# youliangtan/tennisbot-rl

Measured on AMD Instinct MI355X. Metric: env steps/sec (whole node), SwingRacket-v0 @4096 envs/GPU, higher is better.
Workload: dtype f32

## Files before the change

include/tb_stepper.h:

```cpp
#ifndef TB_STEPPER_H
#define TB_STEPPER_H

#include <stddef.h>
#include <stdint.h>

#ifdef __cplusplus
extern "C" {
#endif

#define TB_ABI_VERSION 4

#define TB_OK 0
#define TB_E_INVAL (-1)
#define TB_E_NODEVICE (-2)
#define TB_E_PARAMS (-3)
#define TB_E_UNSUPPORTED (-4)
#define TB_E_TIMEOUT (-5)

#define TB_ENV_SWING 0
#define TB_ENV_TENNIS 1

#define TB_SWING_ACT_DIM 6
#define TB_SWING_OBS_DIM 6
#define TB_TENNIS_ACT_DIM 2
// ... 220 lines not shown
                   long long n_rows, const int64_t *idx_dev, int batch, const float *actor_dev, const float *target_dev,
                   const float *log_ent_coef_dev, const float *eps_next_dev, float gamma, float *y_dev, void *workspace_dev,
                   size_t workspace_bytes);
int tb_tqc_critic_grad(int env_kind, int device, void *stream, const float *obs_dev, const float *action_dev, long long n_rows,
                       const int64_t *idx_dev, int batch, const float *critic_dev, const float *y_dev, float *grad_dev,
                       double *stats_dev, void *workspace_dev, size_t workspace_bytes);
int tb_tqc_actor_grad(int env_kind, int device, void *stream, int batch, const float *actor_dev, const float *critic_dev,
                      const float *log_ent_coef_dev, const float *eps_dev, float *actor_grad_dev, float *ent_grad_dev,
                      double *stats_dev, void *workspace_dev, size_t workspace_bytes);

int tb_set_pipeline(TbHandle *h, int enable);
int tb_flush(TbHandle *h, void *stream);
#define TB_MAX_MARKS 64
int tb_mark_enable(TbHandle *h, int on);
int tb_mark_record(TbHandle *h, int k, void *stream);
int tb_mark_begin(TbHandle *h);
int tb_mark_host_wait(TbHandle *h, int k, int timeout_ms);
long long tb_mark_count(TbHandle *h, int k);
int tb_pipeline_sync(TbHandle *h, int host_wait);
int tb_phase(TbHandle *h);
int tb_phase_advance(TbHandle *h, int n_steps);
int tb_pipeline_form(TbHandle *h);
int tb_step_waves(TbHandle *h);
int tb_pipeline_recover(TbHandle *h);

int tb_get_state(TbHandle *h, uint32_t *words, uint8_t *done, int on_device, void *stream);
int tb_set_state(TbHandle *h, const uint32_t *words, const uint8_t *done, int on_device, void *stream);

#define TB_N_COUNTERS 9
int tb_counters(TbHandle *h, uint64_t *out, void *stream);
int tb_counters_reset(TbHandle *h, void *stream);
int tb_sealed_substeps(TbHandle *h, uint64_t *out, void *stream);

int tb_diag_stream_copy(const uint32_t *src_dev, uint32_t *dst_dev, int n, int rows, int device, void *stream);
int tb_diag_idle(int waves, int microseconds, int device, void *stream);
int tb_diag_two_wave_gate(TbHandle *h, uint8_t *out_dev, void *stream);
int tb_diag_fail_alloc(int nth);

#ifdef __cplusplus
}
#endif
#endif
```

tennisbot_rl_amd/csrc/tb_es.hpp:

```cpp
#pragma once

namespace {

template <int KIND> struct EsNet {
  static constexpr int O = Dims<KIND>::O, A = Dims<KIND>::A, C0 = 8, C1 = 12;
  static constexpr int W0 = 0, B0 = W0 + C0 * O * 2, G0W = B0 + C0, G0B = G0W + C0 * O * 2;
  static constexpr int W1 = G0B + C0, B1 = W1 + C1 * C0 * 2, G1W = B1 + C1, G1B = G1W + C1 * C0 * 2;
  static constexpr int W2 = G1B + C1, B2 = W2 + A * C1 * 2, P = B2 + A;
  static constexpr int PP = (P + 3) / 4 * 4;
  static constexpr int R_X = 0, R_H0 = O, R_H1 = O + 3 * C0, RING = O + 3 * C0 + 5 * C1;
};
template <int KIND> constexpr int es_floats() { return EsNet<KIND>::P; }
static_assert(EsNet<TB_ENV_SWING>::P == 766 && EsNet<TB_ENV_TENNIS>::P == 858, "GatedCNN parameter counts of the reference");
constexpr int TB_ES_LDS_MEMBERS = 8;

constexpr bool es_rows_in_registers(int kind, bool rg) { return kind == TB_ENV_TENNIS && !rg; }
constexpr int es_lds_words(int kind, bool rg) { return lds_words(!es_rows_in_registers(kind, rg), rg); }

struct EsArgs {
  const float* weights;
  size_t stride;
  int per_member;
  double* ret;
  int32_t* len;
// ... 95 lines not shown
  }
  stage_hull(s_hull, A.hull, A.P.n_hull);
  __syncthreads();
  const int m = (live ? i : last) / E.per_member;
  const float* W = staged ? s_w + (m - m0) * N::PP : E.weights + (size_t)m * E.stride;
  float* ring = s_ring + lane;

  EnvRegs e;
  idle_env(e);
  if (live) load_env<KIND>(A.words, A.done_state, A.n, i, e);
  Manifold M;
  init_manifold(M, lane, 64, !es_rows_in_registers(KIND, RG));
  uint32_t cnt[TB_N_COUNTERS] = {};
  KParams Pl = A.P;
  double nrm = 0.0, mean[NO], mdiff[NO];
#pragma unroll
  for (int k = 0; k < NO; ++k) { mean[k] = 0.0; mdiff[k] = 0.0; }
  float o[NO];
  make_obs<KIND>(e, o);
  bool active = live;
  double ret = 0.0;
  int len = 0;
  constexpr unsigned FORM = (RG ? SF_RG : 0u) | SF_COLD | SF_WIDE | (es_rows_in_registers(KIND, RG) ? SF_REGROWS : 0u);
  for (int t = 0; t < T_MAX && __ballot(active) != 0ull; ++t) {
    float a[NA];
#pragma unroll
    for (int k = 0; k < NA; ++k) a[k] = 0.0f;
    const bool rec = active && t < E.t_max;
    if (active) {
      float x[NO], raw[NA];
      es_normalise<NO>(nrm, mean, mdiff, o, x);
      es_net_step<KIND>(W, x, ring, t, raw);
#pragma unroll
      for (int k = 0; k < NA; ++k) a[k] = clip_action(raw[k]);
      if (rec) {
        const size_t row = (size_t)t * A.n + i;
#pragma unroll
        for (int k = 0; k < NO; ++k) { E.t_net_in[row * NO + k] = x[k]; E.t_obs[row * NO + k] = o[k]; }
#pragma unroll
        for (int k = 0; k < NA; ++k) { E.t_act[row * NA + k] = a[k]; E.t_raw[row * NA + k] = raw[k]; }
      }
    }
    int ns = 1;
    bool d = false, parked = false;
    float rew;
    if (KIND == TB_ENV_SWING) rew = swing_step<FORM>(Pl, s_hull, e, M, a, ns, cnt, true, parked TB_STAMP_PASS);
    else rew = tennis_step<FORM>(Pl, s_hull, e, M, a, o, d, cnt TB_STAMP_PASS);
    if (active) {
      end_agent_step<KIND, RG, false>(A, i, e, M, parked, ns, (size_t)i, o, d, cnt);
      if (parked) rew = 0.0f;
      else ret += (double)rew;
      len = t + 1;
      if (rec) {
        E.t_rew[(size_t)t * A.n + i] = rew;
        E.t_done[(size_t)t * A.n + i] = d ? 1 : 0;
      }
      if (d) {
        cnt[5]++;
        active = false;
        idle_env(e);
        M.n = 0; M.deep = 0;
      }
    }
  }
  if (live) { E.ret[i] = ret; E.len[i] = len; }
  flush_counters(A.counters, cnt);
}

__global__ void __launch_bounds__(256) tb_es_fold_kernel(const float* rew_last, double* ret, int n, float* t_rew) {
  const int i = blockIdx.x * blockDim.x + threadIdx.x;
  if (i >= n) return;
  const float r = rew_last[i];
  ret[i] += (double)r;
  if (t_rew) t_rew[(size_t)25 * n + i] = r;
}

}
```

tennisbot_rl_amd/csrc/tb_kernels.hpp:

```cpp
#pragma once
#include <hip/hip_runtime.h>
#include <math.h>

#include "../../include/tb_stepper.h"
#include "tb_device.hpp"
using namespace tb;

namespace {

#define TB_COUNTER_SHARDS 64

struct KArgs {
  KParams P;
  uint32_t* words;
  uint8_t* done_state;
  const float4* hull;
  const float* actions;
  float* obs;
  float* reward;
  uint8_t* done_out;
  float* term_obs;
  int32_t* substeps;
  const uint8_t* mask;
  unsigned long long* counters;
// ... 41 lines not shown
}

template <int KIND> struct Dims;
template <> struct Dims<TB_ENV_SWING> { static constexpr int W = TB_SWING_WORDS, A = TB_SWING_ACT_DIM, O = TB_SWING_OBS_DIM, NAUX = 6; };
template <> struct Dims<TB_ENV_TENNIS> { static constexpr int W = TB_TENNIS_WORDS, A = TB_TENNIS_ACT_DIM, O = TB_TENNIS_OBS_DIM, NAUX = 4; };

template <bool OFF32>
TB_DEV uint32_t row_word(const uint32_t* w, int row, int n, int i) {
  if constexpr (OFF32) {
    const uint32_t byte = ((uint32_t)row * (uint32_t)n + (uint32_t)i) * 4u;
    return *reinterpret_cast<const uint32_t*>(reinterpret_cast<const char*>(w) + byte);
  } else return w[(size_t)row * n + i];
}
template <bool OFF32>
TB_DEV void row_store(uint32_t* w, int row, int n, int i, uint32_t v) {
  if constexpr (OFF32) {
    const uint32_t byte = ((uint32_t)row * (uint32_t)n + (uint32_t)i) * 4u;
    *reinterpret_cast<uint32_t*>(reinterpret_cast<char*>(w) + byte) = v;
  } else w[(size_t)row * n + i] = v;
}
template <int KIND> constexpr bool off32() { return KIND == TB_ENV_SWING; }
template <int KIND> TB_DEV float ld(const uint32_t* w, int row, int n, int i) { return __uint_as_float(row_word<off32<KIND>()>(w, row, n, i)); }
template <int KIND> TB_DEV void st(uint32_t* w, int row, int n, int i, float v) { row_store<off32<KIND>()>(w, row, n, i, __float_as_uint(v)); }

template <int KIND>
TB_DEV void load_env(const uint32_t* w, const uint8_t* done_state, int n, int i, EnvRegs& e) {
  e.r.p = mk(ld<KIND>(w, TB_W_RP, n, i), ld<KIND>(w, TB_W_RP + 1, n, i), ld<KIND>(w, TB_W_RP + 2, n, i));
  e.r.q.x = ld<KIND>(w, TB_W_RQ, n, i); e.r.q.y = ld<KIND>(w, TB_W_RQ + 1, n, i); e.r.q.z = ld<KIND>(w, TB_W_RQ + 2, n, i); e.r.q.w = ld<KIND>(w, TB_W_RQ + 3, n, i);
  e.r.v = mk(ld<KIND>(w, TB_W_RV, n, i), ld<KIND>(w, TB_W_RV + 1, n, i), ld<KIND>(w, TB_W_RV + 2, n, i));
  e.r.w = mk(ld<KIND>(w, TB_W_RW, n, i), ld<KIND>(w, TB_W_RW + 1, n, i), ld<KIND>(w, TB_W_RW + 2, n, i));
  e.b.p = mk(ld<KIND>(w, TB_W_BP, n, i), ld<KIND>(w, TB_W_BP + 1, n, i), ld<KIND>(w, TB_W_BP + 2, n, i));
  e.b.v = mk(ld<KIND>(w, TB_W_BV, n, i), ld<KIND>(w, TB_W_BV + 1, n, i), ld<KIND>(w, TB_W_BV + 2, n, i));
  e.b.w = mk(ld<KIND>(w, TB_W_BW, n, i), ld<KIND>(w, TB_W_BW + 1, n, i), ld<KIND>(w, TB_W_BW + 2, n, i));
#pragma unroll
  for (int k = 0; k < 6; ++k) e.aux[k] = k < Dims<KIND>::NAUX ? ld<KIND>(w, 22 + k, n, i) : 0.0f;
  e.step_count = (int)row_word<off32<KIND>()>(w, Dims<KIND>::W - 2, n, i);
  e.episode = row_word<off32<KIND>()>(w, Dims<KIND>::W - 1, n, i);
  e.done = done_state[i];
}

template <int KIND>
TB_DEV void store_env(uint32_t* w, uint8_t* done_state, int n, int i, const EnvRegs& e, bool all) {
  st<KIND>(w, TB_W_RP, n, i, e.r.p.x); st<KIND>(w, TB_W_RP + 1, n, i, e.r.p.y); st<KIND>(w, TB_W_RP + 2, n, i, e.r.p.z);
  st<KIND>(w, TB_W_RQ, n, i, e.r.q.x); st<KIND>(w, TB_W_RQ + 1, n, i, e.r.q.y); st<KIND>(w, TB_W_RQ + 2, n, i, e.r.q.z); st<KIND>(w, TB_W_RQ + 3, n, i, e.r.q.w);
  st<KIND>(w, TB_W_RV, n, i, e.r.v.x); st<KIND>(w, TB_W_RV + 1, n, i, e.r.v.y); st<KIND>(w, TB_W_RV + 2, n, i, e.r.v.z);
  st<KIND>(w, TB_W_RW, n, i, e.r.w.x); st<KIND>(w, TB_W_RW + 1, n, i, e.r.w.y); st<KIND>(w, TB_W_RW + 2, n, i, e.r.w.z);
// ... 394 lines not shown

TB_DEV void load_ball_side(const uint32_t* w, const uint8_t* done_state, int n, int i, EnvRegs& e) {
  constexpr int K = TB_ENV_SWING;
  e.r.p = mk(ld<K>(w, TB_W_RP, n, i), ld<K>(w, TB_W_RP + 1, n, i), ld<K>(w, TB_W_RP + 2, n, i));
  e.r.q.x = ld<K>(w, TB_W_RQ, n, i); e.r.q.y = ld<K>(w, TB_W_RQ + 1, n, i); e.r.q.z = ld<K>(w, TB_W_RQ + 2, n, i); e.r.q.w = ld<K>(w, TB_W_RQ + 3, n, i);
  e.b.p = mk(ld<K>(w, TB_W_BP, n, i), ld<K>(w, TB_W_BP + 1, n, i), ld<K>(w, TB_W_BP + 2, n, i));
  e.b.v = mk(ld<K>(w, TB_W_BV, n, i), ld<K>(w, TB_W_BV + 1, n, i), ld<K>(w, TB_W_BV + 2, n, i));
  e.b.w = mk(ld<K>(w, TB_W_BW, n, i), ld<K>(w, TB_W_BW + 1, n, i), ld<K>(w, TB_W_BW + 2, n, i));
  e.aux[0] = ld<K>(w, 22, n, i); e.aux[1] = ld<K>(w, 23, n, i);
  e.step_count = (int)row_word<true>(w, Dims<K>::W - 2, n, i);
  e.done = done_state[i];
}
TB_DEV bool two_wave_rare(const KParams& P, const EnvRegs& e) {
  bool rare = e.done != TB_DONE_NO || e.step_count >= 25;
  const vec3 d = e.b.p - e.r.p;
  if ((P.flags & TB_F_RACKET_BALL) && racket_in_reach(P, d, 1.0f)) {
    vec3 ql;
    float qax;
    rare |= racket_slab<false>(P, rotate_inv(e.r.q, d), 1.0f, ql, qax);
  }
  rare |= !(ball_low_point(P, e.b) >= P.static_top + 1.0e-3f);
  return rare;
}
TB_DEV bool two_wave_step(const KArgs& A, const EnvRegs& e, const float* a, int i, bool live TB_DIAG_T0_ARG) {
  constexpr int K = TB_ENV_SWING;
  const KParams& P = A.P;
  const bool racket_wave = threadIdx.x < 64;
  const int lane = (int)(threadIdx.x & 63);
  __shared__ float2 s_rp[64];
  __shared__ float s_ball_fin[64];
  __shared__ int s_rare;
  [[maybe_unused]] const int mk0 = racket_wave ? 0 : 8;
  TB_DIAG_WAIT_LOADS(live);
  TB_DIAG_MARK(mk0);
  if (__any(live && (e.done != TB_DONE_NO || e.step_count >= 25))) return false;
  if (racket_wave) {
    TB_DIAG_MARK(mk0 + 1);
    Racket r = e.r;
    const vec3 F = mk(a[0] * 400.0f, a[1] * 400.0f, FMA(a[2], 400.0f, 4.0f * 9.81f));
    const vec3 T = mk(a[3] * 5.0f, a[4] * 5.0f, a[5] * 5.0f);
    const float speed_r = sqrtf(dot(r.v, r.v));
    racket_velocity(P, r, F, T, rotate_inv(r.q, r.w), speed_r);
    r.p = fma3(P.dt, r.v, r.p);
    s_rp[lane] = make_float2(r.p.x, r.p.y);
    racket_orientation(P, r);
    TB_DIAG_MARK(mk0 + 2);
    asm volatile("s_waitcnt lgkmcnt(0)\n\ts_barrier" ::: "memory");
    TB_DIAG_MARK(mk0 + 3);
    if (__builtin_amdgcn_readfirstlane(s_rare)) return false;
    uint32_t cnt[TB_N_COUNTERS] = {};
    if (live) {
      st<K>(A.words, TB_W_RP, A.n, i, r.p.x); st<K>(A.words, TB_W_RP + 1, A.n, i, r.p.y); st<K>(A.words, TB_W_RP + 2, A.n, i, r.p.z);
      st<K>(A.words, TB_W_RQ, A.n, i, r.q.x); st<K>(A.words, TB_W_RQ + 1, A.n, i, r.q.y); st<K>(A.words, TB_W_RQ + 2, A.n, i, r.q.z);
      st<K>(A.words, TB_W_RQ + 3, A.n, i, r.q.w);
      st<K>(A.words, TB_W_RV, A.n, i, r.v.x); st<K>(A.words, TB_W_RV + 1, A.n, i, r.v.y); st<K>(A.words, TB_W_RV + 2, A.n, i, r.v.z);
      st<K>(A.words, TB_W_RW, A.n, i, r.w.x); st<K>(A.words, TB_W_RW + 1, A.n, i, r.w.y); st<K>(A.words, TB_W_RW + 2, A.n, i, r.w.z);
      float a0 = r.p.x * 0.0f, a1 = r.p.y * 0.0f, a2 = r.p.z * 0.0f, a3 = r.q.x * 0.0f;
      a0 = FMA(r.q.y, 0.0f, a0); a1 = FMA(r.q.z, 0.0f, a1); a2 = FMA(r.q.w, 0.0f, a2); a3 = FMA(r.v.x, 0.0f, a3);
      a0 = FMA(r.v.y, 0.0f, a0); a1 = FMA(r.v.z, 0.0f, a1); a2 = FMA(r.w.x, 0.0f, a2); a3 = FMA(r.w.y, 0.0f, a3);
      a0 = FMA(r.w.z, 0.0f, a0);
      const float t = (a0 + a1) + (a2 + a3);
      if (!(t == t && s_ball_fin[lane] != 0.0f)) cnt[7]++;
    }
    flush_counters(A.counters, cnt);
    TB_DIAG_MARK(mk0 + 4);
  } else {
    Ball b = e.b;
    const float speed_b = sqrtf(dot(b.v, b.v)), spin_b = sqrtf(dot(b.w, b.w));
    ball_velocity(P, b, mk(0.0f, 0.0f, 0.0f), speed_b, spin_b);
    b.p = fma3(P.dt, b.v, b.p);
    float a0 = b.p.x * 0.0f, a1 = b.p.y * 0.0f, a2 = b.p.z * 0.0f, a3 = b.v.x * 0.0f;
    a0 = FMA(b.v.y, 0.0f, a0); a1 = FMA(b.v.z, 0.0f, a1); a2 = FMA(b.w.x, 0.0f, a2); a3 = FMA(b.w.y, 0.0f, a3);
    a0 = FMA(b.w.z, 0.0f, a0);
    const float t = (a0 + a1) + (a2 + a3);
    s_ball_fin[lane] = t == t ? 1.0f : 0.0f;
    const bool rare = __any(live && two_wave_rare(P, e));
    if (lane == 0) s_rare = rare ? 1 : 0;
    TB_DIAG_MARK(mk0 + 1);
    TB_DIAG_MARK(mk0 + 2);
    asm volatile("s_waitcnt lgkmcnt(0)\n\ts_barrier" ::: "memory");
    TB_DIAG_MARK(mk0 + 3);
    if (rare) return false;
    if (live) {
      st<K>(A.words, TB_W_BP, A.n, i, b.p.x); st<K>(A.words, TB_W_BP + 1, A.n, i, b.p.y); st<K>(A.words, TB_W_BP + 2, A.n, i, b.p.z);
      st<K>(A.words, TB_W_BV, A.n, i, b.v.x); st<K>(A.words, TB_W_BV + 1, A.n, i, b.v.y); st<K>(A.words, TB_W_BV + 2, A.n, i, b.v.z);
      st<K>(A.words, TB_W_BW, A.n, i, b.w.x); st<K>(A.words, TB_W_BW + 1, A.n, i, b.w.y); st<K>(A.words, TB_W_BW + 2, A.n, i, b.w.z);
      row_store<true>(A.words, Dims<K>::W - 2, A.n, i, (uint32_t)(e.step_count + 1));
      float2* o = reinterpret_cast<float2*>(A.obs + (size_t)i * 6);
      o[0] = s_rp[lane]; o[1] = make_float2(b.p.x, b.p.y); o[2] = make_float2(e.aux[0], e.aux[1]);
      A.reward[i] = 0.0f;
      A.done_out[i] = 0;
      if (A.substeps) A.substeps[i] = 1;
    }
    TB_DIAG_MARK(mk0 + 4);
  }
  TB_DIAG_ADD_LANE0(mk0 + 5, 1);
  return true;
}

__global__ void __launch_bounds__(64) tb_diag_two_wave_gate_kernel(KArgs A, uint8_t* out) {
  const int i = blockIdx.x * 64 + threadIdx.x;
  if (i >= A.n) return;
  EnvRegs e;
  load_env<TB_ENV_SWING>(A.words, A.done_state, A.n, i, e);
  out[i] = two_wave_rare(A.P, e) ? 1 : 0;
}

}
#include "tb_policy.hpp"
namespace {

#ifndef TB_HINT_TENNIS_CONSTANTS
#define TB_HINT_TENNIS_CONSTANTS 1
#endif
#ifndef TB_HINT_TENNIS_OUTPUTS
#define TB_HINT_TENNIS_OUTPUTS 1
#endif
#ifndef TB_HINT_POLICY_VGPR_PARAMS
#define TB_HINT_POLICY_VGPR_PARAMS 1
#endif
constexpr bool step_rows_in_registers(int kind, bool lean, bool multi, bool rg, bool policy) { return !rg && (kind == TB_ENV_TENNIS || (lean && !multi && !policy)); }
constexpr bool step_has_two_waves(int kind, bool lean, bool multi, bool rg, bool policy) { return kind == TB_ENV_SWING && lean && !multi && !rg && !policy; }
constexpr int step_lds_words(int kind, bool lean, bool multi, bool rg, bool policy) { return lds_words(!step_rows_in_registers(kind, lean, multi, rg, policy), rg); }
template <int KIND, bool LEAN, bool MULTI, bool RG, bool POLICY = false, bool TWO_WAVE = false, int NET = TB_NET_DEFAULT>
__global__ void __launch_bounds__(256) tb_step_kernel(const uint32_t* __restrict__ k_words, const uint8_t* __restrict__ k_done, const float* __restrict__ k_actions,
                                                      const float4* __restrict__ k_hull, int k_n, int k_nhull, KArgs A) {
  constexpr int NA = Dims<KIND>::A, NO = Dims<KIND>::O;
  constexpr bool TABLE_IN_MEMORY = !POLICY && !MULTI && KIND == TB_ENV_TENNIS;
  static_assert(!TWO_WAVE || step_has_two_waves(KIND, LEAN, MULTI, RG, POLICY), "the two-wave form is the pipelined SwingRacket one-step kernel's");
  constexpr bool REGROWS = step_rows_in_registers(KIND, LEAN, MULTI, RG, POLICY);
  constexpr bool LAZYTAB = !POLICY && !MULTI && KIND == TB_ENV_SWING && LEAN && !RG;
  constexpr unsigned FORM = (RG ? SF_RG : 0u) | (REGROWS ? SF_REGROWS : 0u) | (LAZYTAB ? SF_LAZYTAB : 0u);
  __shared__ float4 s_lds_hull[TABLE_IN_MEMORY ? 1 : TB_HULL_LDS];
  __shared__ __attribute__((aligned(16))) float s_mean[POLICY ? 64 * 8 : 4];
  const int i = POLICY || TWO_WAVE ? blockIdx.x * 64 + (threadIdx.x & 63) : blockIdx.x * blockDim.x + threadIdx.x;
  constexpr bool SEP = KIND == TB_ENV_TENNIS;
  const uint32_t* __restrict__ w_words = SEP ? k_words : A.words;
  const uint8_t* __restrict__ w_done = SEP ? k_done : A.done_state;
  const float* __restrict__ w_actions = SEP ? k_actions : A.actions;
  const float4* __restrict__ w_hull = SEP ? k_hull : A.hull;
  const int w_n = SEP ? k_n : A.n, w_nhull = SEP ? k_nhull : A.P.n_hull;
  const float4* const s_hull = TABLE_IN_MEMORY ? w_hull : s_lds_hull;
  const bool live = i < w_n;
  EnvRegs e;
  TB_DIAG_NOW(t_entry);
  TB_DIAG_TRACE_ENTRY(trace_slot);
  TB_DIAG_CADENCE_ENTRY(cad_t0, cad_n);
  float a[NA];
  if (live && !(POLICY && threadIdx.x >= 64)) {
    if (TWO_WAVE && threadIdx.x >= 64) {
      load_ball_side(w_words, w_done, w_n, i, e);
    } else {
      load_env<KIND>(w_words, w_done, w_n, i, e);
      if (!POLICY) load_actions<KIND>(w_actions, (size_t)i, a);
    }
  }
  if constexpr (TWO_WAVE) {
    if (two_wave_step(A, e, a, i, live TB_DIAG_T0_PASS)) {
      TB_DIAG_TRACE_EXIT(trace_slot);
      TB_DIAG_CADENCE_EXIT(cad_t0, cad_n);
      return;
    }
    if (threadIdx.x >= 64) return;
  }
#if TB_HINT_TENNIS_CONSTANTS
  if constexpr (KIND == TB_ENV_TENNIS && !POLICY && !MULTI) {
    asm volatile("" :: "s"(A.P.dt), "s"(A.P.gravity), "s"(A.P.lin_damp), "s"(A.P.lin_damp_quad), "s"(A.P.racket_inv_mass), "s"(A.P.ball_inv_mass),
                 "s"(A.P.hull_bound_radius), "s"(A.P.hull_margin), "s"(A.P.ball_radius), "s"(A.P.contact_threshold), "s"(A.P.static_top), "s"(A.P.max_ang_step));
  }
#endif
#if TB_HINT_TENNIS_OUTPUTS
  if constexpr (KIND == TB_ENV_TENNIS && !POLICY && !MULTI)
    asm volatile("" :: "s"(A.obs), "s"(A.reward), "s"(A.done_out), "s"(A.substeps));
#endif
  Manifold M;
  init_manifold(M, POLICY ? (int)(threadIdx.x & 63) : (int)threadIdx.x, POLICY ? 64 : (int)blockDim.x, !REGROWS);
  const bool had_contacts = load_contacts<RG>(A, i, live && !(POLICY && threadIdx.x >= 64), M);
  if (POLICY) {
    static_assert(TB_HULL_LDS <= 256, "one outline row per thread");
    const bool has_row = (int)threadIdx.x < 2 * w_nhull || ((int)threadIdx.x >= TB_HULL_PLANES && (int)threadIdx.x < TB_HULL_LDS);
    float4 row = make_float4(0.0f, 0.0f, 0.0f, 0.0f);
    if (has_row) row = w_hull[threadIdx.x];
    policy_towers<KIND, NET>(A, s_mean);
    if (has_row) s_lds_hull[threadIdx.x] = row;
    __syncthreads();
    if (threadIdx.x >= 64) return;
// ... 37 lines not shown
      }
      write_obs<KIND>(A.obs, row, o);
      A.reward[row] = rew;
      A.done_out[row] = d ? 1 : 0;
      if constexpr (MULTI && !POLICY) {
        if (t + 1 < n_steps) {
#pragma unroll
          for (int k = 0; k < NA; ++k) a[k] = a_next[k];
        }
      }
    }
    TB_DIAG_ADD_LANE0(15, stamp_now() - t_loaded);
    if (A.substeps) A.substeps[i] = ns_total;
    save_env<KIND, RG>(A, i, e, M, any_reset, had_contacts);
  }
  TB_DIAG_ADD_LANE0(7, t_loaded - t_entry);
  flush_counters(A.counters, cnt);
  TB_DIAG_STAMPS_END(st);
  TB_DIAG_ADD_LANE0(8, stamp_now() - t_kernel0);
  TB_DIAG_ADD_LANE0(9, 1);
  TB_DIAG_ADD_LANE0(14, __builtin_amdgcn_s_memrealtime() - rt_kernel0);
  TB_DIAG_TRACE_EXIT(trace_slot);
  TB_DIAG_CADENCE_EXIT(cad_t0, cad_n);
}

constexpr bool policy_rollout_rows_in_registers(int kind) { return kind == TB_ENV_TENNIS; }
TB_DEV void idle_env(EnvRegs& e) {
  const vec3 z3 = mk(0.0f, 0.0f, 0.0f);
  e.r.p = mk(0.0f, 0.0f, 10.0f); e.r.q.x = 0.0f; e.r.q.y = 0.0f; e.r.q.z = 0.0f; e.r.q.w = 1.0f; e.r.v = z3; e.r.w = z3;
  e.b.p = mk(100.0f, 100.0f, 1000.0f); e.b.v = z3; e.b.w = z3;
#pragma unroll
  for (int k = 0; k < 6; ++k) e.aux[k] = 0.0f;
  e.aux[3] = 1.0f;
  e.aux[5] = 1.0f;
  e.step_count = -(1 << 30); e.episode = 0u; e.done = TB_DONE_NO;
}
constexpr int policy_rollout_lds_words(int kind, bool rg) { return lds_words(!policy_rollout_rows_in_registers(kind), rg); }
template <int KIND, int S, bool RG, int NET = TB_NET_DEFAULT>
__global__ void __launch_bounds__((2 * S + 1) * 64) tb_policy_rollout_kernel(KArgs A) {
  constexpr int NA = Dims<KIND>::A, NO = Dims<KIND>::O, E = TB_POLICY_SLICE * S;
  __shared__ float4 s_hull[TB_HULL_LDS];
  __shared__ __attribute__((aligned(16))) float s_mean[E * 8];
  __shared__ __attribute__((aligned(16))) float s_obs[E * NO];
  const int wave = threadIdx.x >> 6, lane = threadIdx.x & 63;
  stage_hull(s_hull, A.hull, A.P.n_hull);
  if (wave < 2 * S) {
// ... 129 lines not shown
    make_obs<KIND>(e, o);
    if (live) {
#pragma unroll
      for (int k = 0; k < NO; ++k) s_obs[lane * NO + k] = o[k];
    }
  }
  __syncthreads();
  float stdv[NA], lstd[NA];
#pragma unroll
  for (int k = 0; k < NA; ++k) { lstd[k] = A.pol_weights[PolicyBlob<KIND, NET>::LOG_STD + k]; stdv[k] = expf(lstd[k]); }
  KParams Pl = A.P;
#if TB_HINT_POLICY_VGPR_PARAMS
#define TB_PIN(f) asm volatile("" : "+v"(Pl.f))
  TB_PIN(dt); TB_PIN(gravity); TB_PIN(lin_damp); TB_PIN(ang_damp); TB_PIN(lin_damp_quad); TB_PIN(ang_damp_quad); TB_PIN(max_ang_step); TB_PIN(contact_threshold);
  TB_PIN(racket_inv_mass); TB_PIN(racket_inertia[0]); TB_PIN(racket_inertia[1]); TB_PIN(racket_inertia[2]);
  TB_PIN(racket_inv_inertia[0]); TB_PIN(racket_inv_inertia[1]); TB_PIN(racket_inv_inertia[2]);
  TB_PIN(racket_half_thick); TB_PIN(hull_margin); TB_PIN(hull_bound_radius); TB_PIN(ball_inv_mass); TB_PIN(ball_radius); TB_PIN(magnus_k); TB_PIN(static_top);
#undef TB_PIN
#endif
  bool active = live;
  double ret = 0.0;
  int len = 0;
  constexpr unsigned FORM = (RG ? SF_RG : 0u) | SF_COLD | SF_WIDE | (policy_rollout_rows_in_registers(KIND) ? SF_REGROWS : 0u);
  for (int t = 0;; ++t) {
    float eps[NA];
#pragma unroll
    for (int k = 0; k < NA; ++k) eps[k] = 0.0f;
    if (active) policy_draw<KIND>(A, i, e, eps);
    __syncthreads();
    float a[NA], raw[NA], o[NO];
#pragma unroll
    for (int k = 0; k < NA; ++k) { a[k] = 0.0f; raw[k] = 0.0f; }
    if (active) (void)policy_sample_regs<NA>(s_mean + lane * 8, eps, stdv, lstd, raw, a);
    int ns = 1;
    bool d = false, parked = false;
    float rew;
    if (KIND == TB_ENV_SWING) rew = swing_step<FORM>(Pl, s_hull, e, M, a, ns, cnt, true, parked TB_STAMP_PASS);
    else rew = tennis_step<FORM>(Pl, s_hull, e, M, a, o, d, cnt TB_STAMP_PASS);
    if (active) {
      end_agent_step<KIND, RG, false>(A, i, e, M, parked, ns, (size_t)i, o, d, cnt);
      if (!parked) ret += (double)rew;
      len = t + 1;
      if (d) {
        cnt[5]++;
        active = false;
        idle_env(e);
        M.n = 0; M.deep = 0;
      } else {
#pragma unroll
        for (int k = 0; k < NO; ++k) s_obs[lane * NO + k] = o[k];
      }
    }
    const bool go = __ballot(active) != 0ull;
    if (lane == 0) s_go = go ? 1 : 0;
    __syncthreads();
    if (!(t + 1 < T_MAX && __builtin_amdgcn_readfirstlane(s_go) != 0)) break;
  }
  if (live) { ret_out[i] = ret; len_out[i] = len; }
  flush_counters(A.counters, cnt);
}

__global__ void tb_mark_kernel(unsigned long long* count) {
  __hip_atomic_fetch_add(count, 1ull, __ATOMIC_RELAXED, __HIP_MEMORY_SCOPE_SYSTEM);
}

__global__ void tb_poke_kernel(float* dst, float v) { *dst = v; }

constexpr int TB_PHASE_LANES = 64;
constexpr int TB_PHASE_GRID_DIV = 256;
constexpr int TB_BUDGET_MARGIN = 8;
constexpr int ff_lds_words(bool rg, bool esc) { return rows_in_two_slots(esc, rg, false) ? TB_ROWS_LDS_TWO : lds_words(true, rg); }
template <bool RG, bool BIG, bool ESC = false, bool POOL = false>
__global__ void __launch_bounds__(64, (ESC && !RG) ? 4 : 1) tb_ff_kernel(KArgs A) {
  static_assert(!POOL || !ESC, "the pool has no hand-over phase behind it");
  constexpr int TB_FF_REC = ff_rec<RG>();
  __shared__ float4 s_hull[TB_HULL_LDS];
  const int lane = threadIdx.x & 63;
  stage_hull(s_hull, A.hull, A.P.n_hull);
  __syncthreads();
  uint32_t cnt[TB_N_COUNTERS] = {};
  uint32_t n_sealed = 0u;
  TB_DIAG_STAMPS_BEGIN(st);
// ... 124 lines not shown
```

tennisbot_rl_amd/csrc/tb_stepper.hip:

```cpp
#include <hip/hip_runtime.h>
#include <math.h>
#include <stdio.h>
#include <stdlib.h>
#include <string.h>
#include <chrono>

#include "../../include/tb_stepper.h"
#include "tb_device.hpp"

#include "tb_kernels.hpp"
#include "tb_es.hpp"
#include "tb_learner.hpp"
#include "tb_trpo.hpp"
#include "tb_sac.hpp"
#include "tb_tqc.hpp"

using namespace tb;

namespace {

thread_local char g_err[512] = "";

int fail(int code, const char* what) {
  if (code > 0) snprintf(g_err, sizeof g_err, "%s: %s (%s)", what, hipGetErrorString((hipError_t)code), hipGetErrorName((hipError_t)code));
// ... 451 lines not shown
  }
  if (p.slot < 0) return TB_OK;
  a.reward += (size_t)(a.T - 1) * reward_step_stride;
  return launch_ff(h, p.slot, a, s);
}

int count_first_substeps(TbHandle* h, int T, hipStream_t s) {
  hipStreamCaptureStatus st;
  if (int rc = capture_status(s, &st)) return rc;
  if (st == hipStreamCaptureStatusNone) h->first_substeps += (unsigned long long)h->n * (unsigned long long)T;
  return TB_OK;
}

struct PolicyIO {
  const float* weights; const float* obs_in; float* actions; float* raw; float* logp; float* value;
  unsigned long long seed; int deterministic;
  int net;
  void apply(KArgs& a) const {
    a.pol_weights = weights; a.pol_obs = obs_in; a.pol_actions = actions; a.pol_raw = raw; a.pol_logp = logp;
    a.pol_value = value; a.pol_seed = seed; a.pol_deterministic = deterministic;
  }
};

int launch_step(TbHandle* h, int T, const float* actions, float* obs, float* reward, uint8_t* done, float* term, int32_t* substeps, hipStream_t s,
                const PolicyIO* pol = nullptr, bool lean_multi = false) {
  if (int rc = count_first_substeps(h, T, s)) return rc;
  KArgs a = base_args(h);
  if (pol) pol->apply(a);
  a.actions = actions; a.obs = obs; a.reward = reward; a.done_out = done; a.term_obs = term; a.substeps = substeps; a.T = T;
  dim3 grid((unsigned)((h->n + h->block - 1) / h->block)), block((unsigned)h->block);
  if (pol) { grid = dim3((unsigned)((h->n + 63) / 64)); block = dim3(256); }
  const bool piped = (T == 1 || lean_multi) && h->pipeline && h->kind == TB_ENV_SWING && (h->kp.flags & TB_F_AUTO_RESET);
  const bool may_park = piped && ((T == 1 && !h->phase.valid) || h->phase.launch_ends_episode(T));
  Park park;
  if (int rc = claim_park(h, may_park, a, s, &park)) return rc;
  const bool rg = extended_contacts(h->kp);
  const bool multi = T > 1, policy = pol != nullptr;
  const bool two_wave = h->two_wave && step_has_two_waves(h->kind, piped, multi, rg, policy);
  const StepKernel kern = step_kernel(h->kind, piped, multi, rg, policy, two_wave, pol ? pol->net : TB_NET_DEFAULT);
  if (!kern) return fail(TB_E_UNSUPPORTED, "no tb_step_kernel instantiation for this variant");
  if (two_wave) { grid = dim3((unsigned)((h->n + 63) / 64)); block = dim3(128); }
  const size_t lds = dyn_lds(step_lds_words(h->kind, piped, multi, rg, policy), policy ? 64u : block.x);
  (void)hipGetLastError();
  if (int rc = launch(kern, grid, block, lds, s, a.words, a.done_state, a.actions, a.hull, a.n, a.P.n_hull, a)) return rc;
  if (int rc = finish_park(h, park, a, h->n, s)) return rc;
  h->phase.advance(T);
  return TB_OK;
}

int launch_policy_rollout(TbHandle* h, int T, const PolicyIO& pol, float* obs, float* reward, uint8_t* done, const size_t* st ,
                          hipStream_t s) {
  if (int rc = count_first_substeps(h, T, s)) return rc;
  KArgs a = base_args(h);
  pol.apply(a);
  a.obs = obs; a.reward = reward; a.done_out = done; a.T = T;
  a.st_act = st[0]; a.st_raw = st[1]; a.st_logp = st[2]; a.st_val = st[3]; a.st_obs = st[4]; a.st_rew = st[5]; a.st_done = st[6];
  const bool swing = h->kind == TB_ENV_SWING;
  const bool may_park = swing && h->phase.launch_ends_episode(T);
  Park park;
  if (int rc = claim_park(h, may_park, a, s, &park)) return rc;
  const bool narrow = h->opt.policy_slices ? h->opt.policy_slices == 1 : h->n <= 4096;
  const int E = narrow ? TB_POLICY_SLICE : 3 * TB_POLICY_SLICE;
// ... 191 lines not shown

int tb_flush(TbHandle* h, void* stream) {
  if (!h) return fail(TB_E_INVAL, "tb_flush: null handle");
  DeviceGuard g(h->device);
  return flush_all(h, (hipStream_t)stream);
}

int tb_phase(TbHandle* h) {
  if (!h) return fail(TB_E_INVAL, "tb_phase: null handle");
  return h->phase.valid ? h->phase.at : -1;
}

int tb_pipeline_form(TbHandle* h) {
  if (!h) return fail(TB_E_INVAL, "tb_pipeline_form: null handle");
  if (h->kind != TB_ENV_SWING || !h->pipeline) return 0;
  const int mode = defer_mode(h);
  return mode == 2 ? 3 : mode == 1 && h->ff_phases == 1 ? 2 : 1;
}

int tb_step_waves(TbHandle* h) {
  if (!h) return fail(TB_E_INVAL, "tb_step_waves: null handle");
  if (h->kind != TB_ENV_SWING || !h->pipeline) return 0;
  return h->two_wave ? 2 : 1;
}

int tb_phase_advance(TbHandle* h, int n_steps) {
  if (!h || n_steps < 0) return fail(TB_E_INVAL, "tb_phase_advance: bad argument");
  h->phase.advance(n_steps);
  h->first_substeps += (unsigned long long)h->n * (unsigned long long)n_steps;
  return TB_OK;
}

int tb_mark_record(TbHandle* h, int k, void* stream) {
  if (!h || k < 0 || k >= TB_MAX_MARKS) return fail(TB_E_INVAL, "tb_mark_record: bad handle or mark index");
  DeviceGuard g(h->device);
  hipStream_t s = (hipStream_t)stream;
  if (!h->marks.on) return fail(TB_E_UNSUPPORTED, "tb_mark_record needs tb_mark_enable(h, 1) before the steps it covers (their fast-forwards must be counted)");
  hipStreamCaptureStatus st;
  if (int rc = capture_status(s, &st)) return rc;
  if (int rc = run_pool_for_mark(h, s)) return rc;
  if (int rc = launch(tb_mark_kernel, dim3(1), dim3(1), 0, s, h->marks.h + k)) return rc;
  h->marks.in_capture[k] = st == hipStreamCaptureStatusActive;
  for (int q = 0; q < TB_FF_SLOTS; ++q) h->marks.ff_before[k][q] = h->marks.in_capture[k] ? h->slots.s[q].in_capture : h->slots.s[q].eager;
  return TB_OK;
}

// ... 889 lines not shown
```

tennisbot_rl_amd/stepper.py:

```python
import ctypes
import os

import numpy as np

from .params import (ACT_DIM, COUNTER_NAMES, ENV_SWING, ENV_TENNIS, F_AUTO_RESET, N_COUNTERS, NET_DEFAULT, NET_TUNED, OBS_DIM,
                     STATE_ROWS, STATE_WORDS, TbOptions, TbParams, default_params, make_options)

_LIB_PATH = os.path.join(os.path.dirname(os.path.abspath(__file__)), "libtb_stepper.so")
_LIB = None
ABI_VERSION = 4

ENV_IDS = {"SwingRacket-v0": ENV_SWING, "Tennisbot-v0": ENV_TENNIS}


class StepperError(RuntimeError):
    pass


def lib_path():
    return _LIB_PATH


def use_library(path):
    global _LIB_PATH, _LIB
# ... 99 lines not shown
    L.tb_sac_targets.argtypes = [i32, i32, vp, vp, vp, vp, i64, vp, i32, vp, vp, vp, vp, f32, vp, vp, ctypes.c_size_t]
    L.tb_sac_targets.restype = i32
    L.tb_sac_critic_grad.argtypes = [i32, i32, vp, vp, vp, i64, vp, i32, vp, vp, vp, vp, vp, ctypes.c_size_t]
    L.tb_sac_critic_grad.restype = i32
    L.tb_sac_actor_grad.argtypes = [i32, i32, vp, i32, vp, vp, vp, vp, vp, vp, vp, vp, ctypes.c_size_t]
    L.tb_sac_actor_grad.restype = i32
    L.tb_sac_adam.argtypes = [i32, vp, vp, vp, vp, vp, i64, f32, f32, f32, f32, i64, vp, f32]
    L.tb_sac_adam.restype = i32
    L.tb_tqc_param_floats.argtypes = [i32, i32]
    L.tb_tqc_param_floats.restype = i32
    L.tb_tqc_workspace_bytes.argtypes = [i32, i32]
    L.tb_tqc_workspace_bytes.restype = i64
    for sac, tqc in ((L.tb_sac_actor_forward, L.tb_tqc_actor_forward), (L.tb_sac_targets, L.tb_tqc_targets), (L.tb_sac_critic_grad, L.tb_tqc_critic_grad),
                     (L.tb_sac_actor_grad, L.tb_tqc_actor_grad)):
        tqc.argtypes, tqc.restype = sac.argtypes, i32
    L.tb_phase.argtypes = [vp]
    L.tb_phase.restype = i32
    L.tb_phase_advance.argtypes = [vp, i32]
    L.tb_phase_advance.restype = i32
    L.tb_pipeline_form.argtypes = [vp]
    L.tb_pipeline_form.restype = i32
    L.tb_step_waves.argtypes = [vp]
    L.tb_step_waves.restype = i32
    L.tb_params_generation.argtypes = [vp]
    L.tb_params_generation.restype = i32
    L.tb_set_racket_scale.argtypes = [vp, ctypes.c_float, vp]
    L.tb_set_racket_scale.restype = i32
    L.tb_pipeline_recover.argtypes = [vp]
    L.tb_pipeline_recover.restype = i32
    L.tb_mark_record.argtypes = [vp, i32, vp]
    L.tb_mark_record.restype = i32
    L.tb_mark_count.argtypes = [vp, i32]
    L.tb_mark_count.restype = ctypes.c_longlong
    L.tb_mark_host_wait.argtypes = [vp, i32, i32]
    L.tb_mark_host_wait.restype = i32
    L.tb_mark_begin.argtypes = [vp]
    L.tb_mark_begin.restype = i32
    L.tb_mark_enable.argtypes = [vp, i32]
    L.tb_mark_enable.restype = i32
    L.tb_diag_stream_copy.argtypes = [vp, vp, i32, i32, i32, vp]
    L.tb_diag_stream_copy.restype = i32
    L.tb_diag_idle.argtypes = [i32, i32, i32, vp]
    L.tb_diag_idle.restype = i32
    L.tb_diag_two_wave_gate.argtypes = [vp, vp, vp]
    L.tb_diag_two_wave_gate.restype = i32
    L.tb_diag_fail_alloc.argtypes = [i32]
# ... 364 lines not shown
        return f[rows].t().contiguous()

    def set_params(self, params):
        p = params.copy()
        p.flags = (p.flags | F_AUTO_RESET) if self.auto_reset else (p.flags & ~F_AUTO_RESET)
        _check(self.L, self.L.tb_set_params(self._h, ctypes.byref(p), self._stream()), "tb_set_params")
        self.params = p

    def set_racket_scale(self, scale):
        _check(self.L, self.L.tb_set_racket_scale(self._h, float(scale), self._stream()), "tb_set_racket_scale")
        self.params.racket_scale = float(scale)

    def phase(self):
        return int(self.L.tb_phase(self._h))

    PIPELINE_FORMS = ("none", "slots", "slots+pool", "pool")

    def pipeline_form(self):
        return self.PIPELINE_FORMS[int(self.L.tb_pipeline_form(self._h))]

    def step_waves(self):
        return int(self.L.tb_step_waves(self._h))

    def get_state_words(self):
        t = self.torch
        w = t.empty((self.words, self.num_envs), dtype=t.int32, device=self.device)
        d = t.empty(self.num_envs, dtype=t.uint8, device=self.device)
        _check(self.L, self.L.tb_get_state(self._h, w.data_ptr(), d.data_ptr(), 1, self._stream()), "tb_get_state")
        return w, d

    def set_state_words(self, words, done=None):
        t = self.torch
        w = words if isinstance(words, t.Tensor) else t.from_numpy(np.ascontiguousarray(words).view(np.int32))
        w = self._check_tensor(w.to(self.device).contiguous(), (self.words, self.num_envs), t.int32, "words")
        dptr = None
        if done is not None:
            d = done if isinstance(done, t.Tensor) else t.from_numpy(np.ascontiguousarray(done, np.uint8))
            d = self._check_tensor(d.to(self.device).contiguous(), (self.num_envs,), t.uint8, "done")
            dptr = d.data_ptr()
        _check(self.L, self.L.tb_set_state(self._h, w.data_ptr(), dptr, 1, self._stream()), "tb_set_state")
        self.torch.cuda.current_stream(self.device).synchronize()

    def get_state(self):
        w, d = self.get_state_words()
        w = w.cpu().numpy().view(np.uint32)
        names = STATE_ROWS[self.kind]
# ... 39 lines not shown
```

Baseline: 945.0 million.

## Add short two-wave step form that skips episode-end gate using host phase tracking

Adds a SHORT variant of the two-wave SwingRacket step kernel, chosen when the host-tracked phase shows the launch cannot end an episode. The kernel then drops the upfront full-state load and done/step-count ballot gate. Each wave instead loads only its own rows, using precomputed byte offsets, and the kernel args are re-fetched late so fewer registers stay live. The aim is to cut latency and register pressure in the common mid-episode step, at the cost of relying on the host phase being correct and on one more kernel instantiation.

```diff
diff --git a/include/tb_stepper.h b/include/tb_stepper.h
--- a/include/tb_stepper.h
+++ b/include/tb_stepper.h
@@ -266,6 +266,7 @@
 int tb_phase_advance(TbHandle *h, int n_steps);
 int tb_pipeline_form(TbHandle *h);
 int tb_step_waves(TbHandle *h);
+int tb_step_form(TbHandle *h);
 int tb_pipeline_recover(TbHandle *h);
 
 int tb_get_state(TbHandle *h, uint32_t *words, uint8_t *done, int on_device, void *stream);
diff --git a/tennisbot_rl_amd/csrc/tb_es.hpp b/tennisbot_rl_amd/csrc/tb_es.hpp
--- a/tennisbot_rl_amd/csrc/tb_es.hpp
+++ b/tennisbot_rl_amd/csrc/tb_es.hpp
@@ -141,6 +141,7 @@
   double ret = 0.0;
   int len = 0;
   constexpr unsigned FORM = (RG ? SF_RG : 0u) | SF_COLD | SF_WIDE | (es_rows_in_registers(KIND, RG) ? SF_REGROWS : 0u);
+  TB_DIAG_STAMPS_BEGIN(st);
   for (int t = 0; t < T_MAX && __ballot(active) != 0ull; ++t) {
     float a[NA];
 #pragma unroll
@@ -184,6 +185,7 @@
   }
   if (live) { E.ret[i] = ret; E.len[i] = len; }
   flush_counters(A.counters, cnt);
+  TB_DIAG_STAMPS_END(st);
 }
 
 __global__ void __launch_bounds__(256) tb_es_fold_kernel(const float* rew_last, double* ret, int n, float* t_rew) {
diff --git a/tennisbot_rl_amd/csrc/tb_kernels.hpp b/tennisbot_rl_amd/csrc/tb_kernels.hpp
--- a/tennisbot_rl_amd/csrc/tb_kernels.hpp
+++ b/tennisbot_rl_amd/csrc/tb_kernels.hpp
@@ -87,6 +87,15 @@
 template <int KIND> constexpr bool off32() { return KIND == TB_ENV_SWING; }
 template <int KIND> TB_DEV float ld(const uint32_t* w, int row, int n, int i) { return __uint_as_float(row_word<off32<KIND>()>(w, row, n, i)); }
 template <int KIND> TB_DEV void st(uint32_t* w, int row, int n, int i, float v) { row_store<off32<KIND>()>(w, row, n, i, __float_as_uint(v)); }
+TB_DEV uint32_t row_byte(int row, int n, int i) {
+  uint32_t byte = ((uint32_t)row * (uint32_t)n + (uint32_t)i) * 4u;
+  asm("" : "+v"(byte));
+  return byte;
+}
+TB_DEV uint32_t word_at(const uint32_t* w, uint32_t byte) { return *reinterpret_cast<const uint32_t*>(reinterpret_cast<const char*>(w) + byte); }
+TB_DEV void word_to(uint32_t* w, uint32_t byte, uint32_t v) { *reinterpret_cast<uint32_t*>(reinterpret_cast<char*>(w) + byte) = v; }
+TB_DEV float ld_at(const uint32_t* w, uint32_t byte) { return __uint_as_float(word_at(w, byte)); }
+TB_DEV void st_at(uint32_t* w, uint32_t byte, float v) { word_to(w, byte, __float_as_uint(v)); }
 
 template <int KIND>
 TB_DEV void load_env(const uint32_t* w, const uint8_t* done_state, int n, int i, EnvRegs& e) {
@@ -527,8 +536,11 @@
   rare |= !(ball_low_point(P, e.b) >= P.static_top + 1.0e-3f);
   return rare;
 }
-TB_DEV bool two_wave_step(const KArgs& A, const EnvRegs& e, const float* a, int i, bool live TB_DIAG_T0_ARG) {
+template <bool SHORT>
+TB_DEV bool two_wave_step(const KArgs& A, EnvRegs& e, float* a, int i, bool live TB_DIAG_T0_ARG) {
   constexpr int K = TB_ENV_SWING;
+  static_assert(TB_W_RQ == TB_W_RP + 3 && TB_W_RV == TB_W_RP + 7 && TB_W_RW == TB_W_RP + 10 && TB_W_BV == TB_W_BP + 3 && TB_W_BW == TB_W_BP + 6,
+                "the racket's 13 rows and the ball's 9 are consecutive");
   const KParams& P = A.P;
   const bool racket_wave = threadIdx.x < 64;
   const int lane = (int)(threadIdx.x & 63);
@@ -536,12 +548,30 @@
   __shared__ float s_ball_fin[64];
   __shared__ int s_rare;
   [[maybe_unused]] const int mk0 = racket_wave ? 0 : 8;
-  TB_DIAG_WAIT_LOADS(live);
-  TB_DIAG_MARK(mk0);
-  if (__any(live && (e.done != TB_DONE_NO || e.step_count >= 25))) return false;
+  if constexpr (!SHORT) {
+    TB_DIAG_WAIT_LOADS(live);
+    TB_DIAG_MARK(mk0);
+    if (__any(live && (e.done != TB_DONE_NO || e.step_count >= 25))) return false;
+  }
   if (racket_wave) {
+    Racket r;
+    [[maybe_unused]] uint32_t at[13];
+    if constexpr (SHORT) {
+#pragma unroll
+      for (int k = 0; k < 13; ++k) at[k] = row_byte(TB_W_RP + k, A.n, i);
+      if (live) {
+        load_actions<K>(A.actions, (size_t)i, a);
+        r.w = mk(ld_at(A.words, at[10]), ld_at(A.words, at[11]), ld_at(A.words, at[12]));
+        r.q.x = ld_at(A.words, at[3]); r.q.y = ld_at(A.words, at[4]); r.q.z = ld_at(A.words, at[5]); r.q.w = ld_at(A.words, at[6]);
+        r.v = mk(ld_at(A.words, at[7]), ld_at(A.words, at[8]), ld_at(A.words, at[9]));
+        r.p = mk(ld_at(A.words, at[0]), ld_at(A.words, at[1]), ld_at(A.words, at[2]));
+      }
+      TB_DIAG_WAIT_LOADS(live);
+      TB_DIAG_MARK(mk0);
+    } else {
+      r = e.r;
+    }
     TB_DIAG_MARK(mk0 + 1);
-    Racket r = e.r;
     const vec3 F = mk(a[0] * 400.0f, a[1] * 400.0f, FMA(a[2], 400.0f, 4.0f * 9.81f));
     const vec3 T = mk(a[3] * 5.0f, a[4] * 5.0f, a[5] * 5.0f);
     const float speed_r = sqrtf(dot(r.v, r.v));
@@ -555,11 +585,12 @@
     if (__builtin_amdgcn_readfirstlane(s_rare)) return false;
     uint32_t cnt[TB_N_COUNTERS] = {};
     if (live) {
-      st<K>(A.words, TB_W_RP, A.n, i, r.p.x); st<K>(A.words, TB_W_RP + 1, A.n, i, r.p.y); st<K>(A.words, TB_W_RP + 2, A.n, i, r.p.z);
-      st<K>(A.words, TB_W_RQ, A.n, i, r.q.x); st<K>(A.words, TB_W_RQ + 1, A.n, i, r.q.y); st<K>(A.words, TB_W_RQ + 2, A.n, i, r.q.z);
-      st<K>(A.words, TB_W_RQ + 3, A.n, i, r.q.w);
-      st<K>(A.words, TB_W_RV, A.n, i, r.v.x); st<K>(A.words, TB_W_RV + 1, A.n, i, r.v.y); st<K>(A.words, TB_W_RV + 2, A.n, i, r.v.z);
-      st<K>(A.words, TB_W_RW, A.n, i, r.w.x); st<K>(A.words, TB_W_RW + 1, A.n, i, r.w.y); st<K>(A.words, TB_W_RW + 2, A.n, i, r.w.z);
+      const float out[13] = {r.p.x, r.p.y, r.p.z, r.q.x, r.q.y, r.q.z, r.q.w, r.v.x, r.v.y, r.v.z, r.w.x, r.w.y, r.w.z};
+#pragma unroll
+      for (int k = 0; k < 13; ++k) {
+        if constexpr (SHORT) st_at(A.words, at[k], out[k]);
+        else st<K>(A.words, TB_W_RP + k, A.n, i, out[k]);
+      }
       float a0 = r.p.x * 0.0f, a1 = r.p.y * 0.0f, a2 = r.p.z * 0.0f, a3 = r.q.x * 0.0f;
       a0 = FMA(r.q.y, 0.0f, a0); a1 = FMA(r.q.z, 0.0f, a1); a2 = FMA(r.q.w, 0.0f, a2); a3 = FMA(r.v.x, 0.0f, a3);
       a0 = FMA(r.v.y, 0.0f, a0); a1 = FMA(r.v.z, 0.0f, a1); a2 = FMA(r.w.x, 0.0f, a2); a3 = FMA(r.w.y, 0.0f, a3);
@@ -570,6 +601,25 @@
     flush_counters(A.counters, cnt);
     TB_DIAG_MARK(mk0 + 4);
   } else {
+    [[maybe_unused]] uint32_t at[10];
+    if constexpr (SHORT) {
+#pragma unroll
+      for (int k = 0; k < 9; ++k) at[k] = row_byte(TB_W_BP + k, A.n, i);
+      at[9] = row_byte(Dims<K>::W - 2, A.n, i);
+      if (live) {
+        const uint32_t* w = A.words;
+        e.r.p = mk(ld<K>(w, TB_W_RP, A.n, i), ld<K>(w, TB_W_RP + 1, A.n, i), ld<K>(w, TB_W_RP + 2, A.n, i));
+        e.r.q.x = ld<K>(w, TB_W_RQ, A.n, i); e.r.q.y = ld<K>(w, TB_W_RQ + 1, A.n, i); e.r.q.z = ld<K>(w, TB_W_RQ + 2, A.n, i); e.r.q.w = ld<K>(w, TB_W_RQ + 3, A.n, i);
+        e.b.p = mk(ld_at(w, at[0]), ld_at(w, at[1]), ld_at(w, at[2]));
+        e.b.v = mk(ld_at(w, at[3]), ld_at(w, at[4]), ld_at(w, at[5]));
+        e.b.w = mk(ld_at(w, at[6]), ld_at(w, at[7]), ld_at(w, at[8]));
+        e.aux[0] = ld<K>(w, 22, A.n, i); e.aux[1] = ld<K>(w, 23, A.n, i);
+        e.step_count = (int)word_at(w, at[9]);
+        e.done = A.done_state[i];
+      }
+      TB_DIAG_WAIT_LOADS(live);
+      TB_DIAG_MARK(mk0);
+    }
     Ball b = e.b;
     const float speed_b = sqrtf(dot(b.v, b.v)), spin_b = sqrtf(dot(b.w, b.w));
     ball_velocity(P, b, mk(0.0f, 0.0f, 0.0f), speed_b, spin_b);
@@ -587,10 +637,14 @@
     TB_DIAG_MARK(mk0 + 3);
     if (rare) return false;
     if (live) {
-      st<K>(A.words, TB_W_BP, A.n, i, b.p.x); st<K>(A.words, TB_W_BP + 1, A.n, i, b.p.y); st<K>(A.words, TB_W_BP + 2, A.n, i, b.p.z);
-      st<K>(A.words, TB_W_BV, A.n, i, b.v.x); st<K>(A.words, TB_W_BV + 1, A.n, i, b.v.y); st<K>(A.words, TB_W_BV + 2, A.n, i, b.v.z);
-      st<K>(A.words, TB_W_BW, A.n, i, b.w.x); st<K>(A.words, TB_W_BW + 1, A.n, i, b.w.y); st<K>(A.words, TB_W_BW + 2, A.n, i, b.w.z);
-      row_store<true>(A.words, Dims<K>::W - 2, A.n, i, (uint32_t)(e.step_count + 1));
+      const float out[9] = {b.p.x, b.p.y, b.p.z, b.v.x, b.v.y, b.v.z, b.w.x, b.w.y, b.w.z};
+#pragma unroll
+      for (int k = 0; k < 9; ++k) {
+        if constexpr (SHORT) st_at(A.words, at[k], out[k]);
+        else st<K>(A.words, TB_W_BP + k, A.n, i, out[k]);
+      }
+      if constexpr (SHORT) word_to(A.words, at[9], (uint32_t)(e.step_count + 1));
+      else row_store<true>(A.words, Dims<K>::W - 2, A.n, i, (uint32_t)(e.step_count + 1));
       float2* o = reinterpret_cast<float2*>(A.obs + (size_t)i * 6);
       o[0] = s_rp[lane]; o[1] = make_float2(b.p.x, b.p.y); o[2] = make_float2(e.aux[0], e.aux[1]);
       A.reward[i] = 0.0f;
@@ -627,12 +681,20 @@
 constexpr bool step_rows_in_registers(int kind, bool lean, bool multi, bool rg, bool policy) { return !rg && (kind == TB_ENV_TENNIS || (lean && !multi && !policy)); }
 constexpr bool step_has_two_waves(int kind, bool lean, bool multi, bool rg, bool policy) { return kind == TB_ENV_SWING && lean && !multi && !rg && !policy; }
 constexpr int step_lds_words(int kind, bool lean, bool multi, bool rg, bool policy) { return lds_words(!step_rows_in_registers(kind, lean, multi, rg, policy), rg); }
-template <int KIND, bool LEAN, bool MULTI, bool RG, bool POLICY = false, bool TWO_WAVE = false, int NET = TB_NET_DEFAULT>
+struct StepKernelArgs { const uint32_t* words; const uint8_t* done; const float* actions; const float4* hull; int n, n_hull; KArgs A; };
+TB_DEV const KArgs* refetched_args() {
+  auto seg = (const __attribute__((address_space(4))) char*)__builtin_amdgcn_kernarg_segment_ptr();
+  asm volatile("" : "+s"(seg));
+  return (const KArgs*)(seg + offsetof(StepKernelArgs, A));
+}
+template <int KIND, bool LEAN, bool MULTI, bool RG, bool POLICY = false, bool TWO_WAVE = false, int NET = TB_NET_DEFAULT, bool SHORT = false>
 __global__ void __launch_bounds__(256) tb_step_kernel(const uint32_t* __restrict__ k_words, const uint8_t* __restrict__ k_done, const float* __restrict__ k_actions,
-                                                      const float4* __restrict__ k_hull, int k_n, int k_nhull, KArgs A) {
+                                                      const float4* __restrict__ k_hull, int k_n, int k_nhull, KArgs k_args) {
+  const KArgs& A = k_args;
   constexpr int NA = Dims<KIND>::A, NO = Dims<KIND>::O;
   constexpr bool TABLE_IN_MEMORY = !POLICY && !MULTI && KIND == TB_ENV_TENNIS;
   static_assert(!TWO_WAVE || step_has_two_waves(KIND, LEAN, MULTI, RG, POLICY), "the two-wave form is the pipelined SwingRacket one-step kernel's");
+  static_assert(!SHORT || TWO_WAVE, "the short form is a two-wave form");
   constexpr bool REGROWS = step_rows_in_registers(KIND, LEAN, MULTI, RG, POLICY);
   constexpr bool LAZYTAB = !POLICY && !MULTI && KIND == TB_ENV_SWING && LEAN && !RG;
   constexpr unsigned FORM = (RG ? SF_RG : 0u) | (REGROWS ? SF_REGROWS : 0u) | (LAZYTAB ? SF_LAZYTAB : 0u);
@@ -652,7 +714,7 @@
   TB_DIAG_TRACE_ENTRY(trace_slot);
   TB_DIAG_CADENCE_ENTRY(cad_t0, cad_n);
   float a[NA];
-  if (live && !(POLICY && threadIdx.x >= 64)) {
+  if (!SHORT && live && !(POLICY && threadIdx.x >= 64)) {
     if (TWO_WAVE && threadIdx.x >= 64) {
       load_ball_side(w_words, w_done, w_n, i, e);
     } else {
@@ -661,12 +723,21 @@
     }
   }
   if constexpr (TWO_WAVE) {
-    if (two_wave_step(A, e, a, i, live TB_DIAG_T0_PASS)) {
+    if (two_wave_step<SHORT>(A, e, a, i, live TB_DIAG_T0_PASS)) {
       TB_DIAG_TRACE_EXIT(trace_slot);
       TB_DIAG_CADENCE_EXIT(cad_t0, cad_n);
       return;
     }
     if (threadIdx.x >= 64) return;
+  }
+  const KArgs* late_args = &k_args;
+  if constexpr (SHORT) late_args = refetched_args();
+  {
+  const KArgs& A = *late_args;
+  const float4* __restrict__ w_hull = SEP ? k_hull : A.hull;
+  const int w_nhull = SEP ? k_nhull : A.P.n_hull;
+  if constexpr (SHORT) {
+    if (live) load_env<KIND>(A.words, A.done_state, A.n, i, e);
   }
 #if TB_HINT_TENNIS_CONSTANTS
   if constexpr (KIND == TB_ENV_TENNIS && !POLICY && !MULTI) {
@@ -750,6 +821,7 @@
   TB_DIAG_ADD_LANE0(14, __builtin_amdgcn_s_memrealtime() - rt_kernel0);
   TB_DIAG_TRACE_EXIT(trace_slot);
   TB_DIAG_CADENCE_EXIT(cad_t0, cad_n);
+  }
 }
 
 constexpr bool policy_rollout_rows_in_registers(int kind) { return kind == TB_ENV_TENNIS; }
@@ -925,6 +997,7 @@
   double ret = 0.0;
   int len = 0;
   constexpr unsigned FORM = (RG ? SF_RG : 0u) | SF_COLD | SF_WIDE | (policy_rollout_rows_in_registers(KIND) ? SF_REGROWS : 0u);
+  TB_DIAG_STAMPS_BEGIN(st);
   for (int t = 0;; ++t) {
     float eps[NA];
 #pragma unroll
@@ -961,6 +1034,7 @@
   }
   if (live) { ret_out[i] = ret; len_out[i] = len; }
   flush_counters(A.counters, cnt);
+  TB_DIAG_STAMPS_END(st);
 }
 
 __global__ void tb_mark_kernel(unsigned long long* count) {
diff --git a/tennisbot_rl_amd/csrc/tb_stepper.hip b/tennisbot_rl_amd/csrc/tb_stepper.hip
--- a/tennisbot_rl_amd/csrc/tb_stepper.hip
+++ b/tennisbot_rl_amd/csrc/tb_stepper.hip
@@ -497,6 +497,13 @@
   }
 };
 
+enum { TB_STEP_ONE_WAVE = 0, TB_STEP_TWO_WAVE_GATE = 1, TB_STEP_TWO_WAVE_SHORT = 2 };
+int step_form(const TbHandle* h, bool lean, bool multi, bool rg, bool policy) {
+  if (!h->two_wave || !step_has_two_waves(h->kind, lean, multi, rg, policy)) return TB_STEP_ONE_WAVE;
+  if (!h->phase.valid) return TB_STEP_TWO_WAVE_GATE;
+  return h->phase.launch_ends_episode(1) ? TB_STEP_ONE_WAVE : TB_STEP_TWO_WAVE_SHORT;
+}
+
 int launch_step(TbHandle* h, int T, const float* actions, float* obs, float* reward, uint8_t* done, float* term, int32_t* substeps, hipStream_t s,
                 const PolicyIO* pol = nullptr, bool lean_multi = false) {
   if (int rc = count_first_substeps(h, T, s)) return rc;
@@ -511,8 +518,10 @@
   if (int rc = claim_park(h, may_park, a, s, &park)) return rc;
   const bool rg = extended_contacts(h->kp);
   const bool multi = T > 1, policy = pol != nullptr;
-  const bool two_wave = h->two_wave && step_has_two_waves(h->kind, piped, multi, rg, policy);
-  const StepKernel kern = step_kernel(h->kind, piped, multi, rg, policy, two_wave, pol ? pol->net : TB_NET_DEFAULT);
+  const int form = step_form(h, piped, multi, rg, policy);
+  const bool two_wave = form != TB_STEP_ONE_WAVE;
+  const StepKernel kern = form == TB_STEP_TWO_WAVE_SHORT ? tb_step_kernel<TB_ENV_SWING, true, false, false, false, true, TB_NET_DEFAULT, true>
+                                                         : step_kernel(h->kind, piped, multi, rg, policy, two_wave, pol ? pol->net : TB_NET_DEFAULT);
   if (!kern) return fail(TB_E_UNSUPPORTED, "no tb_step_kernel instantiation for this variant");
   if (two_wave) { grid = dim3((unsigned)((h->n + 63) / 64)); block = dim3(128); }
   const size_t lds = dyn_lds(step_lds_words(h->kind, piped, multi, rg, policy), policy ? 64u : block.x);
@@ -750,6 +759,12 @@
   if (!h) return fail(TB_E_INVAL, "tb_step_waves: null handle");
   if (h->kind != TB_ENV_SWING || !h->pipeline) return 0;
   return h->two_wave ? 2 : 1;
+}
+
+int tb_step_form(TbHandle* h) {
+  if (!h) return fail(TB_E_INVAL, "tb_step_form: null handle");
+  if (h->kind != TB_ENV_SWING || !h->pipeline || !(h->kp.flags & TB_F_AUTO_RESET)) return -1;
+  return step_form(h, true, false, extended_contacts(h->kp), false);
 }
 
 int tb_phase_advance(TbHandle* h, int n_steps) {
diff --git a/tennisbot_rl_amd/stepper.py b/tennisbot_rl_amd/stepper.py
--- a/tennisbot_rl_amd/stepper.py
+++ b/tennisbot_rl_amd/stepper.py
@@ -145,6 +145,8 @@
     L.tb_pipeline_form.restype = i32
     L.tb_step_waves.argtypes = [vp]
     L.tb_step_waves.restype = i32
+    L.tb_step_form.argtypes = [vp]
+    L.tb_step_form.restype = i32
     L.tb_params_generation.argtypes = [vp]
     L.tb_params_generation.restype = i32
     L.tb_set_racket_scale.argtypes = [vp, ctypes.c_float, vp]
@@ -555,6 +557,9 @@
     def step_waves(self):
         return int(self.L.tb_step_waves(self._h))
 
+    def step_form(self):
+        return int(self.L.tb_step_form(self._h))
+
     def get_state_words(self):
         t = self.torch
         w = t.empty((self.words, self.num_envs), dtype=t.int32, device=self.device)
```

Measured after the change: 980.1 million (median of 6 runs). 3.7% higher.
